# ppjian19/PhoreGen

Hardware: AMD Instinct MI355X
Metric: denoise-steps/sec (batch=128, ~40-atom graphs) (higher is better)
Workload: dtype f32; 1 GPU; BASELINE.json configs[2]: ONE batch of 128 LigPhore-shaped graphs (n~N(40,6) atoms, p~N(107,30) pharmacophore nodes), partitioned over 1 GPU(s) by the fitted step cost, steps t=999.. of the 1000-step sampler, device Philox noise, trajectory written; graphs_total=128, graphs_rank0=128, n_ctx=18401, n_lig=5115, e_knn=588832, e_bond=203720, e3=8087028, parallelism=graph-sharded x1, final RCCL gather only, triplet_workgroups_rank0=256

## Files before the change

### phoregen_amd/csrc/triplet2.hip

```cpp
#include "wave_prims.h"
#include "triplet2_rows.h"
#include "../../include/phoregen_hip.h"

namespace pg {

#ifdef PG_T2_PROF
#define T2_STAMP(slot) do { const unsigned long long t2_now = __builtin_amdgcn_s_memtime(); t2_acc[slot] += t2_now - t2_last; t2_last = t2_now; } while (0)
#else
#define T2_STAMP(slot) do { } while (0)
#endif

typedef float t2_f2 __attribute__((ext_vector_type(2)));

#ifdef PG_DEGRADE_BITS
#define T2_DEGRADE(v) __builtin_bit_cast(float, __builtin_bit_cast(unsigned, (v)) & (0xffffffffu << PG_DEGRADE_BITS))
#else
#define T2_DEGRADE(v) (v)
#endif

constexpr int T2_ROW = 260;
constexpr int T2_ROWS = PG_SEG_TRI_STAGED_ROWS;
constexpr int T2_XS = PG_SEG_TRI_STAGED_ATOMS;

constexpr size_t t2_lds_floats() { return 16384 + 2 * 1536 + 3 * 128 + 3 * T2_XS + 4 + (size_t)T2_ROWS * T2_ROW; }

template <int THREADS, int MAXT, bool TRAIN = false>
__global__ __launch_bounds__(THREADS) void triplet2_kernel(PgTopo t, PgSegAttn p) {
  constexpr bool PRE = THREADS <= 512;
  constexpr int WAVES = THREADS / 64;
  extern __shared__ __attribute__((aligned(16))) float lds[];
  float* const w2k_l = lds;
  float* const wf_k = w2k_l + 16384;
  float* const wf_v = wf_k + 1536;
  float* const bk = wf_v + 1536;
  float* const bv = bk + 128;
  float* const b2v = bv + 128;
  float* const xs = b2v + 128;
  int* const ctrl = reinterpret_cast<int*>(xs + 3 * T2_XS);
  float* const pbuf = xs + 3 * T2_XS + 4;
  const int tid = threadIdx.x, lane = tid & 63;
  const int wave = __builtin_amdgcn_readfirstlane(tid >> 6);
  const int g = lane >> 4, m = lane & 15;

  for (int i = tid; i < 128; i += THREADS) { bk[i] = p.ln_bk[i]; bv[(i & 15) * 8 + (i >> 4)] = p.ln_bv[i]; b2v[i] = TRAIN ? 0.f : p.b2v[i]; }
  for (int i = tid; i < 1536; i += THREADS) {
    const int ln_ = i & 63, tq_ = (i >> 6) & 7, st_ = i >> 9;
    const int d_ = ((st_ * 2 + (tq_ >> 2)) * 64 + ln_) * 4 + (tq_ & 3);
    wf_k[d_] = p.Wf_k[i]; wf_v[d_] = p.Wf_v[i];
  }
  for (int i = tid; i < 4096; i += THREADS) reinterpret_cast<f4*>(w2k_l)[i] = reinterpret_cast<const f4*>(p.W2k_l)[i];
  const f4* const w2v_g = reinterpret_cast<const f4*>(p.W2v_l);
  const int4* const iters = reinterpret_cast<const int4*>(p.tri_iters);
#ifdef PG_T2_PROF
  unsigned long long t2_acc[8] = {0, 0, 0, 0, 0, 0, 0, 0};
  unsigned long long t2_last = __builtin_amdgcn_s_memtime();
#endif

  for (;;) {
    __syncthreads();
    if (tid == 0) ctrl[0] = atomicAdd(p.tri_counter, 1);
    __syncthreads();
    const int it = __builtin_amdgcn_readfirstlane(ctrl[0]);
    T2_STAMP(0);
    if (it >= p.n_tri_iters) {
      if (tid == 0 && atomicAdd(p.tri_counter + 1, 1) == (int)gridDim.x - 1) {
        p.tri_counter[0] = 0;
        p.tri_counter[1] = 0;
        __threadfence();
      }
      break;
    }
    const int4 d = iters[it];
    const int lig0 = __builtin_amdgcn_readfirstlane(d.x);
    const int n = __builtin_amdgcn_readfirstlane(d.y & 0xff), j0 = __builtin_amdgcn_readfirstlane((d.y >> 8) & 0xff);
    const int A = __builtin_amdgcn_readfirstlane(d.y >> 16), bond_off = __builtin_amdgcn_readfirstlane(d.z);
    const int nm1 = n - 1;
    {
      const f4* src = reinterpret_cast<const f4*>(p.Csrc_k + (size_t)(bond_off + j0 * nm1) * 256);
      const int n4 = A * nm1 * 64;
      for (int idx = tid; idx < n4; idx += THREADS)
        *reinterpret_cast<f4*>(pbuf + (idx >> 6) * T2_ROW + (idx & 63) * 4) = __builtin_nontemporal_load(src + idx);
      for (int i = tid; i < n * 3; i += THREADS) xs[i] = p.x[(size_t)lig0 * 3 + i];
    }
    __syncthreads();
    T2_STAMP(1);
    const int s_begin = __builtin_amdgcn_readfirstlane(d.w & 0xffff);
    const int n_seg = __builtin_amdgcn_readfirstlane((d.w >> 16) ? (d.w >> 16) : A * nm1);
    const int nr = nm1 - 1;
    const int n_tiles = (nr + 15) >> 4;
    const int tail_tile = n_tiles - 1;
    const int tail_slices = t2_tail_slices(t2_tail_rows(nr, n_tiles));

    float nQk[8], nQv[8];
    f4 nqa, nqb;
    float2 nrs = {0.f, 0.f};
#define T2_FETCH(S)                                                                                                    \
    {                                                                                                                  \
      const int a_ = (S) / nm1, ip_ = (S) - a_ * nm1, j_ = j0 + a_, i_ = ip_ + (ip_ >= j_ ? 1 : 0);                    \
      const size_t seg_ = (size_t)(bond_off + i_ * nm1 + (j_ < i_ ? j_ : j_ - 1));                                     \
       \
      const float* qp_ = p.q + seg_ * 128 + 8 * m;                                                                     \
      nqa = __builtin_nontemporal_load(reinterpret_cast<const f4*>(qp_));                                              \
      nqb = __builtin_nontemporal_load(reinterpret_cast<const f4*>(qp_ + 4));                                          \
      const float* qk_ = p.Cdst_k + seg_ * p.ld_cdst + m;                                                              \
      const float* qv_ = p.Cdst_v + seg_ * p.ld_cdst + m;                                                              \
      _Pragma("unroll") for (int tq = 0; tq < 8; ++tq) { nQk[tq] = __builtin_nontemporal_load(qk_ + 16 * tq); nQv[tq] = __builtin_nontemporal_load(qv_ + 16 * tq); } \
      if constexpr (!TRAIN) { const t2_f2 r_ = __builtin_nontemporal_load(reinterpret_cast<const t2_f2*>(p.resid + seg_ * 128 + 8 * m + 2 * g)); nrs.x = r_[0]; nrs.y = r_[1]; } \
    }
    if (PRE && s_begin + wave < n_seg) T2_FETCH(s_begin + wave)

    for (int s = s_begin + wave; s < n_seg; s += WAVES) {
      const int a = s / nm1, ip = s - a * nm1;
      const int j = j0 + a, i = ip + (ip >= j ? 1 : 0);
      const int seg = bond_off + i * nm1 + (j < i ? j : j - 1);
      const float* const prow = pbuf + a * nm1 * T2_ROW;
      if (!PRE) T2_FETCH(s)
      float cQk[8], cQv[8];
#pragma unroll
      for (int tq = 0; tq < 8; ++tq) { cQk[tq] = nQk[tq]; cQv[tq] = nQv[tq]; }
      const f4 qa = nqa, qb = nqb;
      const float2 rsd = nrs;
      if (PRE && s + WAVES < n_seg) T2_FETCH(s + WAVES)
      int lz = lane;
      asm volatile("" : "+v"(lz));

      float wk2[8], wv2[8];
#pragma unroll
      for (int tq = 0; tq < 8; ++tq) {
        wk2[tq] = g == 3 ? cQk[tq] : wf_k[((4 + (tq >> 2)) * 64 + lane) * 4 + (tq & 3)];
        wv2[tq] = g == 3 ? cQv[tq] : wf_v[((4 + (tq >> 2)) * 64 + lane) * 4 + (tq & 3)];
      }
      T2_STAMP(2);
      const float xi0 = xs[i * 3], xi1 = xs[i * 3 + 1], xi2 = xs[i * 3 + 2];
      const float u0 = xs[j * 3] - xi0, u1 = xs[j * 3 + 1] - xi1, u2 = xs[j * 3 + 2] - xi2;

      float feat[MAXT][3];
      f4 lg[MAXT];

      float th_own[(MAXT + 3) / 4];
#pragma unroll
      for (int rep = 0; rep < (MAXT + 3) / 4; ++rep) {
        const int kp = (4 * rep + g) * 16 + m;
        const int kq = kp < nr ? kp : 0;
        const int kc = kq + (kq >= ip ? 1 : 0);
        const int k = kc + (kc >= j ? 1 : 0);
        const float v0 = xs[k * 3] - xi0, v1 = xs[k * 3 + 1] - xi1, v2 = xs[k * 3 + 2] - xi2;
        const float dt = u0 * v0 + u1 * v1 + u2 * v2;
        const float c0 = u1 * v2 - u2 * v1, c1 = u2 * v0 - u0 * v2, c2 = u0 * v1 - u1 * v0;
        th_own[rep] = atan2f(sqrtf(c0 * c0 + c1 * c1 + c2 * c2), dt);
      }

      {
        f4 U[8];
        {
#pragma unroll
          for (int tq = 0; tq < 8; ++tq)
#pragma unroll
            for (int r = 0; r < 4; ++r) {
              const int w = (tq * 4 + r) * 2;
              const f4 wa = *reinterpret_cast<const f4*>(w2k_l + ((size_t)w * 64 + lane) * 4);
              const f4 wb = *reinterpret_cast<const f4*>(w2k_l + ((size_t)(w + 1) * 64 + lane) * 4);
              float u = qa[0] * wa[0];
              u = fmaf(qa[1], wa[1], u); u = fmaf(qa[2], wa[2], u); u = fmaf(qa[3], wa[3], u);
              u = fmaf(qb[0], wb[0], u); u = fmaf(qb[1], wb[1], u); u = fmaf(qb[2], wb[2], u); u = fmaf(qb[3], wb[3], u);
              U[tq][r] = u;
            }
        }
#pragma unroll
        for (int slot = 0; slot < MAXT; ++slot) {
          const bool tail = slot == MAXT - 1;
          const int tile = tail ? tail_tile : slot;
          lg[slot] = (f4){NEG_BIG, NEG_BIG, NEG_BIG, NEG_BIG};
          feat[slot][0] = feat[slot][1] = feat[slot][2] = 0.f;
          if (tail ? tail_tile >= 0 : slot < tail_tile) {
            const int mr = t2_tile_row(tail, m);
            const int kp = tile * 16 + mr;
            const int kq = !tail || kp < nr ? kp : 0;
            const int kc = kq + (kq >= ip ? 1 : 0);
            float th_src = th_own[0];
#pragma unroll
            for (int rep = 1; rep < (MAXT + 3) / 4; ++rep) th_src = (tile >> 2) == rep ? th_own[rep] : th_src;
            const float theta = from_lane(th_src, 16 * (tile & 3) + mr);
            float sg, cg;
            sincos_bounded_pair(theta * (g == 0 ? 1.0f : (g == 1 ? 0.5f : (float)(1.0 / 3.0))), sg, cg);
            const float s1 = from_lane(sg, m), c1 = from_lane(cg, m);
            const float sx = from_lane(sg, m + (g == 0 ? 16 : 32));
            feat[slot][0] = g == 0 ? theta : (g == 1 ? s1 : (g == 2 ? 2.0f * s1 * c1 : s1 * fmaf(-4.0f * s1, s1, 3.0f)));
            feat[slot][1] = g < 2 ? sx : (g == 2 ? c1 : fmaf(-2.0f * s1, s1, 1.0f));
            feat[slot][2] = g == 0 ? c1 * fmaf(4.0f * c1, c1, -3.0f) : (g == 3 ? 1.0f : cg);
            f4 hid[8];
            const float* pk = prow + kc * T2_ROW + 4 * g;
#pragma unroll
            for (int tq = 0; tq < 8; ++tq) hid[tq] = *reinterpret_cast<const f4*>(pk + 16 * tq);
#pragma unroll
            for (int st = 0; st < 2; ++st)
              {
                const f4 wa = *reinterpret_cast<const f4*>(wf_k + ((st * 2) * 64 + lane) * 4);
                const f4 wb = *reinterpret_cast<const f4*>(wf_k + ((st * 2 + 1) * 64 + lane) * 4);
#pragma unroll
                for (int tq = 0; tq < 4; ++tq) hid[tq] = mfma16(wa[tq], feat[slot][st], hid[tq]);
#pragma unroll
                for (int tq = 0; tq < 4; ++tq) hid[4 + tq] = mfma16(wb[tq], feat[slot][st], hid[4 + tq]);
              }
#pragma unroll
            for (int tq = 0; tq < 8; ++tq) hid[tq] = mfma16(wk2[tq], feat[slot][2], hid[tq]);
            float q2 = 0.f;
#pragma unroll
            for (int tq = 0; tq < 8; ++tq)
#pragma unroll
              for (int r = 0; r < 4; ++r) q2 = fmaf(hid[tq][r], hid[tq][r], q2);
            q2 += __shfl_xor(q2, 16);
            q2 += __shfl_xor(q2, 32);
            const float var = q2 * (1.f / 128.f) + 1e-5f;
            const float rs = __builtin_amdgcn_rsqf(var);
            const float sigma = var * rs;
            f4 acc4[4];
#pragma unroll
            for (int r = 0; r < 4; ++r) acc4[r] = (f4){0.f, 0.f, 0.f, 0.f};
#pragma unroll
            for (int tq = 0; tq < 8; ++tq) {
              const f4 bt = *reinterpret_cast<const f4*>(bk + 16 * tq + 4 * g);
#pragma unroll
              for (int r = 0; r < 4; ++r) acc4[r] = mfma16(T2_DEGRADE(fmaxf(fmaf(bt[r], sigma, hid[tq][r]), 0.f)), U[tq][r], acc4[r]);
            }
            f4 acc = (acc4[0] + acc4[1]) + (acc4[2] + acc4[3]);
#pragma unroll
            for (int r = 0; r < 4; ++r) acc[r] *= __shfl(rs, 4 * g + r);
#pragma unroll
            for (int r = 0; r < 4; ++r) {
              const int kr = tile * 16 + t2_elem_row(tail, g, r);
              lg[slot][r] = !tail || kr < nr ? acc[r] : NEG_BIG;
            }
          }
        }
      }

      T2_STAMP(3);
      float mx = NEG_BIG;
#pragma unroll
      for (int slot = 0; slot < MAXT; ++slot)
#pragma unroll
        for (int r = 0; r < 4; ++r) mx = fmaxf(mx, lg[slot][r]);
      mx = fmaxf(mx, __shfl_xor(mx, 16));
      mx = fmaxf(mx, __shfl_xor(mx, 32));
      float l = 0.f;
#pragma unroll
      for (int slot = 0; slot < MAXT; ++slot)
#pragma unroll
        for (int r = 0; r < 4; ++r) {
          const float e = lg[slot][r] > 0.5f * NEG_BIG ? __builtin_amdgcn_exp2f(lg[slot][r] - mx) : 0.f;
          lg[slot][r] = e;
          l += e;
        }
      l += __shfl_xor(l, 16);
      l += __shfl_xor(l, 32);
      const float inv = l > 0.f ? 1.0f / l : 0.f;

      if constexpr (TRAIN) {
        if (p.alpha) {
          float* const ap = p.alpha + (size_t)seg * p.alpha_rows * 16 + m;
#pragma unroll
          for (int slot = 0; slot < MAXT; ++slot) {
            const bool tail = slot == MAXT - 1;
            const int tile = tail ? tail_tile : slot;
            if (tail ? tail_tile >= 0 : slot < tail_tile) {
#pragma unroll
              for (int r = 0; r < 4; ++r) {
                const int kr = tile * 16 + t2_elem_row(tail, g, r);
                const int kc = kr + (kr >= ip ? 1 : 0);
                if (!tail || kr < nr) ap[(kc + (kc >= j ? 1 : 0)) * 16] = lg[slot][r] * inv;
              }
            }
          }
          if (g == 0) { ap[j * 16] = 0.f; ap[i * 16] = 0.f; }
        }
      }
      T2_STAMP(4);
      f4 sT[8];
#pragma unroll
      for (int tq = 0; tq < 8; ++tq) sT[tq] = (f4){0.f, 0.f, 0.f, 0.f};
#pragma unroll
      for (int slot = 0; slot < MAXT; ++slot) {
        const bool tail = slot == MAXT - 1;
        const int tile = tail ? tail_tile : slot;
        if (tail ? tail_tile >= 0 : slot < tail_tile) {
          f4 hv[8];
#pragma unroll
          for (int r = 0; r < 4; ++r) {
            if (!tail || r < tail_slices) {
              const int kr = tile * 16 + t2_elem_row(tail, g, r);
              const int kq = !tail || kr < nr ? kr : 0;
              const float* pv = prow + (kq + (kq >= ip ? 1 : 0)) * T2_ROW + 128 + m;
#pragma unroll
              for (int tq = 0; tq < 8; ++tq) hv[tq][r] = pv[16 * tq];
            } else {
#pragma unroll
              for (int tq = 0; tq < 8; ++tq) hv[tq][r] = 0.f;
            }
          }
#pragma unroll
          for (int st = 0; st < 2; ++st)
            {
              const f4 wa = *reinterpret_cast<const f4*>(wf_v + ((st * 2) * 64 + lane) * 4);
              const f4 wb = *reinterpret_cast<const f4*>(wf_v + ((st * 2 + 1) * 64 + lane) * 4);
#pragma unroll
              for (int tq = 0; tq < 4; ++tq) hv[tq] = mfma16(feat[slot][st], wa[tq], hv[tq]);
#pragma unroll
              for (int tq = 0; tq < 4; ++tq) hv[4 + tq] = mfma16(feat[slot][st], wb[tq], hv[4 + tq]);
            }
#pragma unroll
          for (int tq = 0; tq < 8; ++tq) hv[tq] = mfma16(feat[slot][2], wv2[tq], hv[tq]);
          if (!tail) {
            f4 q2 = {0.f, 0.f, 0.f, 0.f};
#pragma unroll
            for (int tq = 0; tq < 8; ++tq) q2 += hv[tq] * hv[tq];
            f4 sg, aw;
#pragma unroll
            for (int r = 0; r < 4; ++r) {
              const float var = row16_total(q2[r]) * (1.f / 128.f) + 1e-5f;
              const float rsq = __builtin_amdgcn_rsqf(var);
              sg[r] = var * rsq;
              aw[r] = lg[slot][r] * rsq;
            }
#pragma unroll
            for (int tq = 0; tq < 8; ++tq) {
              const float bt = bv[m * 8 + tq];
#pragma unroll
              for (int r = 0; r < 4; ++r) hv[tq][r] = T2_DEGRADE(fmaxf(fmaf(bt, sg[r], hv[tq][r]), 0.f));
            }
#pragma unroll
            for (int r = 0; r < 4; ++r)
#pragma unroll
              for (int tq = 0; tq < 8; ++tq) sT[tq] = mfma16(hv[tq][r], aw[r], sT[tq]);
          } else {
            float bt[8];
#pragma unroll
            for (int tq = 0; tq < 8; ++tq) bt[tq] = bv[m * 8 + tq];
#pragma unroll
            for (int r = 0; r < 4; ++r) {
              if (r < tail_slices) {
                float q2 = 0.f;
#pragma unroll
                for (int tq = 0; tq < 8; ++tq) q2 = fmaf(hv[tq][r], hv[tq][r], q2);
                const float var = row16_total(q2) * (1.f / 128.f) + 1e-5f;
                const float rsq = __builtin_amdgcn_rsqf(var);
                const float sg = var * rsq;
                const float aw = lg[slot][r] * rsq;
#pragma unroll
                for (int tq = 0; tq < 8; ++tq) sT[tq] = mfma16(T2_DEGRADE(fmaxf(fmaf(bt[tq], sg, hv[tq][r]), 0.f)), aw, sT[tq]);
              }
            }
          }
        }
      }

      T2_STAMP(5);
      if constexpr (TRAIN) {
        float* const sp = p.S + (size_t)seg * 2048 + lane;
#pragma unroll
        for (int tq = 0; tq < 8; ++tq)
#pragma unroll
          for (int r = 0; r < 4; ++r) sp[(tq * 4 + r) * 64] = sT[tq][r] * inv;
        if (g == 0) p.swn[(size_t)seg * 16 + m] = l > 0.f ? 1.f : 0.f;
        continue;
      }
      const size_t ro = (size_t)seg * 128 + 8 * m + 2 * g;
      float part[8] = {0.f, 0.f, 0.f, 0.f, 0.f, 0.f, 0.f, 0.f};
#pragma unroll
      for (int w = 0; w < 64; ++w) {
        const int tq = w >> 3, r = (w >> 1) & 3, hf = (w & 1) * 4;
        const f4 wv_ = w2v_g[w * 64 + lz];
        const float sv = sT[tq][r];
        part[hf + 0] = fmaf(wv_[0], sv, part[hf + 0]); part[hf + 1] = fmaf(wv_[1], sv, part[hf + 1]);
        part[hf + 2] = fmaf(wv_[2], sv, part[hf + 2]); part[hf + 3] = fmaf(wv_[3], sv, part[hf + 3]);
      }
#pragma unroll
      for (int dd = 0; dd < 8; ++dd) {
        part[dd] += __shfl_xor(part[dd], 16);
        part[dd] += __shfl_xor(part[dd], 32);
      }
      const float has = l > 0.f ? 1.f : 0.f;
      const int o0 = 8 * m + 2 * g;
      const float p0 = g == 0 ? part[0] : (g == 1 ? part[2] : (g == 2 ? part[4] : part[6]));
      const float p1 = g == 0 ? part[1] : (g == 1 ? part[3] : (g == 2 ? part[5] : part[7]));
      float2 o;
      o.x = rsd.x + p0 * inv + b2v[o0] * has;
      o.y = rsd.y + p1 * inv + b2v[o0 + 1] * has;
      __builtin_nontemporal_store((t2_f2){o.x, o.y}, reinterpret_cast<t2_f2*>(p.out + ro));
      T2_STAMP(6);
    }
#undef T2_FETCH
    T2_STAMP(7);
  }
#ifdef PG_T2_PROF
  if (lane == 0 && p.alpha) {
    unsigned long long* prof = reinterpret_cast<unsigned long long*>(p.alpha);
    for (int k = 0; k < 8; ++k) atomicAdd(prof + k, t2_acc[k]);
  }
#endif
}

template <int THREADS, int MAXT, bool TRAIN = false>
static int launch_t2(const PgTopo* t, const PgSegAttn* p, hipStream_t st) {
  const size_t lds = t2_lds_floats() * sizeof(float);
  if (int rc = reserve_lds(reinterpret_cast<const void*>(triplet2_kernel<THREADS, MAXT, TRAIN>), lds, "pg_seg_attn(triplet, staged)")) return rc;
  const int grid = (p->tri_grid > 0 && p->tri_grid < kNumCU) ? p->tri_grid : kNumCU;
  hipLaunchKernelGGL((triplet2_kernel<THREADS, MAXT, TRAIN>), dim3(grid), dim3(THREADS), lds, st, *t, *p);
  return check_launch("pg_seg_attn(triplet, staged)");
}

int launch_triplet_staged(const PgSegForm& f, const PgTopo* t, const PgSegAttn* p, hipStream_t st) {
  const int variant = f.family == PG_FORM_TRI_STAGED_TRAIN ? 2 : f.threads == 512 ? 1 : 0;
  switch (f.tiles * 10 + variant) {
    case 32: return launch_t2<768, 3, true>(t, p, st);
    case 42: return launch_t2<768, 4, true>(t, p, st);
    case 52: return launch_t2<768, 5, true>(t, p, st);
    case 30: return launch_t2<768, 3>(t, p, st);
    case 40: return launch_t2<768, 4>(t, p, st);
    case 50: return launch_t2<768, 5>(t, p, st);
    case 31: return launch_t2<512, 3>(t, p, st);
    case 41: return launch_t2<512, 4>(t, p, st);
    case 51: return launch_t2<512, 5>(t, p, st);
  }
  set_error("pg_seg_attn: no staged triplet instance for %d row tiles", f.tiles);
  return PG_ERR_ARG;
}

}
```

Before: 58.22 steps/s.

## Prefetch next work item inside segment loop and batch LDS staging loads

Moves the work-queue atomic and descriptor fetch for the next iteration into the last segment pass of wave 0, so the pull overlaps compute and one barrier per iteration is removed. The descriptor goes to LDS as an int4, and termination is detected by d.y==0. Weight preloading and per-iteration row staging now issue all global loads into registers before the LDS stores, which exposes memory-level parallelism. The cost is higher register pressure, clamped redundant loads, and reliance on a zero descriptor meaning the queue is done.

```diff
diff --git a/phoregen_amd/csrc/triplet2.hip b/phoregen_amd/csrc/triplet2.hip
--- a/phoregen_amd/csrc/triplet2.hip
+++ b/phoregen_amd/csrc/triplet2.hip
@@ -42,15 +42,38 @@
   const int wave = __builtin_amdgcn_readfirstlane(tid >> 6);
   const int g = lane >> 4, m = lane & 15;
 
-  for (int i = tid; i < 128; i += THREADS) { bk[i] = p.ln_bk[i]; bv[(i & 15) * 8 + (i >> 4)] = p.ln_bv[i]; b2v[i] = TRAIN ? 0.f : p.b2v[i]; }
-  for (int i = tid; i < 1536; i += THREADS) {
-    const int ln_ = i & 63, tq_ = (i >> 6) & 7, st_ = i >> 9;
-    const int d_ = ((st_ * 2 + (tq_ >> 2)) * 64 + ln_) * 4 + (tq_ & 3);
-    wf_k[d_] = p.Wf_k[i]; wf_v[d_] = p.Wf_v[i];
-  }
-  for (int i = tid; i < 4096; i += THREADS) reinterpret_cast<f4*>(w2k_l)[i] = reinterpret_cast<const f4*>(p.W2k_l)[i];
   const f4* const w2v_g = reinterpret_cast<const f4*>(p.W2v_l);
   const int4* const iters = reinterpret_cast<const int4*>(p.tri_iters);
+  static_assert(1536 % THREADS == 0 && THREADS >= 128 && THREADS >= 3 * T2_XS, "fill passes");
+  constexpr int NW2 = (4096 + THREADS - 1) / THREADS, NWF = 1536 / THREADS;
+  constexpr int NST = (T2_ROWS * 64 + THREADS - 1) / THREADS;
+  {
+    int it0 = 0;
+    if (tid == 0) it0 = atomicAdd(p.tri_counter, 1);
+    f4 w2[NW2];
+    float fk[NWF], fv[NWF];
+#pragma unroll
+    for (int k = 0; k < NW2; ++k) { const int i = tid + k * THREADS; w2[k] = reinterpret_cast<const f4*>(p.W2k_l)[i < 4096 ? i : 4095]; }
+#pragma unroll
+    for (int k = 0; k < NWF; ++k) { fk[k] = p.Wf_k[tid + k * THREADS]; fv[k] = p.Wf_v[tid + k * THREADS]; }
+    const int ib = tid & 127;
+    const float lk = p.ln_bk[ib], lv = p.ln_bv[ib];
+    float l2 = 0.f;
+    if constexpr (!TRAIN) l2 = p.b2v[ib];
+    int4 d0 = {0, 0, 0, 0};
+    if (tid == 0 && it0 < p.n_tri_iters) d0 = iters[it0];
+#pragma unroll
+    for (int k = 0; k < NW2; ++k) { const int i = tid + k * THREADS; if (i < 4096) reinterpret_cast<f4*>(w2k_l)[i] = w2[k]; }
+#pragma unroll
+    for (int k = 0; k < NWF; ++k) {
+      const int i = tid + k * THREADS;
+      const int ln_ = i & 63, tq_ = (i >> 6) & 7, st_ = i >> 9;
+      const int d_ = ((st_ * 2 + (tq_ >> 2)) * 64 + ln_) * 4 + (tq_ & 3);
+      wf_k[d_] = fk[k]; wf_v[d_] = fv[k];
+    }
+    if (tid < 128) { bk[tid] = lk; bv[(tid & 15) * 8 + (tid >> 4)] = lv; b2v[tid] = l2; }
+    if (tid == 0) *reinterpret_cast<int4*>(ctrl) = d0;
+  }
 #ifdef PG_T2_PROF
   unsigned long long t2_acc[8] = {0, 0, 0, 0, 0, 0, 0, 0};
   unsigned long long t2_last = __builtin_amdgcn_s_memtime();
@@ -58,11 +81,12 @@
 
   for (;;) {
     __syncthreads();
-    if (tid == 0) ctrl[0] = atomicAdd(p.tri_counter, 1);
-    __syncthreads();
-    const int it = __builtin_amdgcn_readfirstlane(ctrl[0]);
+    const int4 dv = *reinterpret_cast<const int4*>(ctrl);
+    int4 d;
+    d.x = __builtin_amdgcn_readfirstlane(dv.x); d.y = __builtin_amdgcn_readfirstlane(dv.y);
+    d.z = __builtin_amdgcn_readfirstlane(dv.z); d.w = __builtin_amdgcn_readfirstlane(dv.w);
     T2_STAMP(0);
-    if (it >= p.n_tri_iters) {
+    if (d.y == 0) {
       if (tid == 0 && atomicAdd(p.tri_counter + 1, 1) == (int)gridDim.x - 1) {
         p.tri_counter[0] = 0;
         p.tri_counter[1] = 0;
@@ -70,17 +94,31 @@
       }
       break;
     }
-    const int4 d = iters[it];
     const int lig0 = __builtin_amdgcn_readfirstlane(d.x);
     const int n = __builtin_amdgcn_readfirstlane(d.y & 0xff), j0 = __builtin_amdgcn_readfirstlane((d.y >> 8) & 0xff);
     const int A = __builtin_amdgcn_readfirstlane(d.y >> 16), bond_off = __builtin_amdgcn_readfirstlane(d.z);
     const int nm1 = n - 1;
     {
       const f4* src = reinterpret_cast<const f4*>(p.Csrc_k + (size_t)(bond_off + j0 * nm1) * 256);
-      const int n4 = A * nm1 * 64;
-      for (int idx = tid; idx < n4; idx += THREADS)
-        *reinterpret_cast<f4*>(pbuf + (idx >> 6) * T2_ROW + (idx & 63) * 4) = __builtin_nontemporal_load(src + idx);
-      for (int i = tid; i < n * 3; i += THREADS) xs[i] = p.x[(size_t)lig0 * 3 + i];
+      const int n4 = A * nm1 * 64, nx = n * 3;
+      int tz = tid;
+      asm volatile("" : "+v"(tz));
+      f4 rows[NST];
+#pragma unroll
+      for (int k = 0; k < NST; ++k) {
+        const int idx = tz + k * THREADS;
+        rows[k] = __builtin_nontemporal_load(src + (idx < n4 ? idx : n4 - 1));
+      }
+      float xv = p.x[(size_t)lig0 * 3 + (tz < nx ? tz : nx - 1)];
+#pragma unroll
+      for (int k = 0; k < NST; ++k) asm volatile("" : "+v"(rows[k]));
+      asm volatile("" : "+v"(xv));
+#pragma unroll
+      for (int k = 0; k < NST; ++k) {
+        const int idx = tz + k * THREADS;
+        if (idx < n4) *reinterpret_cast<f4*>(pbuf + (idx >> 6) * T2_ROW + (idx & 63) * 4) = rows[k];
+      }
+      if (tz < nx) xs[tz] = xv;
     }
     __syncthreads();
     T2_STAMP(1);
@@ -121,6 +159,9 @@
       const f4 qa = nqa, qb = nqb;
       const float2 rsd = nrs;
       if (PRE && s + WAVES < n_seg) T2_FETCH(s + WAVES)
+      const bool last0 = wave == 0 && s + WAVES >= n_seg;
+      int nit = 0;
+      if (last0 && lane == 0) nit = atomicAdd(p.tri_counter, 1);
       int lz = lane;
       asm volatile("" : "+v"(lz));
 
@@ -236,6 +277,8 @@
       }
 
       T2_STAMP(3);
+      int4 nd = {0, 0, 0, 0};
+      if (last0 && lane == 0 && nit < p.n_tri_iters) nd = iters[nit];
       float mx = NEG_BIG;
 #pragma unroll
       for (int slot = 0; slot < MAXT; ++slot)
@@ -362,6 +405,7 @@
 #pragma unroll
           for (int r = 0; r < 4; ++r) sp[(tq * 4 + r) * 64] = sT[tq][r] * inv;
         if (g == 0) p.swn[(size_t)seg * 16 + m] = l > 0.f ? 1.f : 0.f;
+        if (last0 && lane == 0) *reinterpret_cast<int4*>(ctrl) = nd;
         continue;
       }
       const size_t ro = (size_t)seg * 128 + 8 * m + 2 * g;
@@ -387,9 +431,16 @@
       o.x = rsd.x + p0 * inv + b2v[o0] * has;
       o.y = rsd.y + p1 * inv + b2v[o0 + 1] * has;
       __builtin_nontemporal_store((t2_f2){o.x, o.y}, reinterpret_cast<t2_f2*>(p.out + ro));
+      if (last0 && lane == 0) *reinterpret_cast<int4*>(ctrl) = nd;
       T2_STAMP(6);
     }
 #undef T2_FETCH
+    if (s_begin >= n_seg && tid == 0) {
+      const int nit = atomicAdd(p.tri_counter, 1);
+      int4 nd = {0, 0, 0, 0};
+      if (nit < p.n_tri_iters) nd = iters[nit];
+      *reinterpret_cast<int4*>(ctrl) = nd;
+    }
     T2_STAMP(7);
   }
 #ifdef PG_T2_PROF
```

New measurement: 58.15 steps/s. Within noise of the previous version (-0.1%).
